# apache/incubator-predictionio

Hardware: NVIDIA H100
Metric: ALS iterations/sec (higher is better)
Workload: dtype f32

## Files before the change

### incubator-predictionio_b200/csrc/pio_als.cu

```cuda
#include "../../include/pio_als.h"

#include <cuda_runtime.h>
#include <dlfcn.h>
#include <math.h>
#include <nccl.h>
#include <stdarg.h>
#include <stdio.h>
#include <stdlib.h>
#include <string.h>

#include <chrono>
#include <algorithm>
#include <array>
#include <deque>
#include <exception>
#include <map>
#include <memory>
#include <mutex>
#include <string>
#include <type_traits>
#include <vector>

#include "als_kernels.cuh"
#include "als_mma_kernel.cuh"
#include "als_pair_kernel.cuh"
#define TC_NS tc
#define TC_NTEAM 2
#define TC_NCONV 5
#define TC_NGATHER 2
#define TC_NSTAGE 6
#define TC_NRAW 7
#include "als_tc_kernel.cuh"
#undef TC_NS
#undef TC_NTEAM
#undef TC_NCONV
#undef TC_NGATHER
#undef TC_NSTAGE
#undef TC_NRAW
#include "sort_scan.cuh"
#include "topk.cuh"
#include "score_plan.h"
#include "solve_plan.h"
#include "ids_encode.cuh"
#include "events_scan.cuh"
#include "events_fold.cuh"
#include "events_index.cuh"
#include "cooc.cuh"
#include "cooc_predict.cuh"
#include "popular.cuh"
#include "serve_merge.cuh"
#include "forest.cuh"
#include "eval_folds.cuh"
#include "cls_folds.cuh"

namespace pio {

static thread_local std::string g_create_error;

static int ceil_log2(uint64_t n) {
  int b = 0;
  while (b < 63 && (1ull << b) < n) ++b;
  return b < 1 ? 1 : b;
}
static int pad_rank(int k) { return k <= 16 ? 16 : k <= 32 ? 32 : k <= 64 ? 64 : 128; }

struct NcclApi {
  void* lib = nullptr;
  ncclResult_t (*GetUniqueId)(ncclUniqueId*) = nullptr;
  ncclResult_t (*CommInitRank)(ncclComm_t*, int, ncclUniqueId, int) = nullptr;
  ncclResult_t (*AllGather)(const void*, void*, size_t, ncclDataType_t, ncclComm_t, cudaStream_t) = nullptr;
  ncclResult_t (*AllReduce)(const void*, void*, size_t, ncclDataType_t, ncclRedOp_t, ncclComm_t, cudaStream_t) = nullptr;
  ncclResult_t (*Send)(const void*, size_t, ncclDataType_t, int, ncclComm_t, cudaStream_t) = nullptr;
  ncclResult_t (*Recv)(void*, size_t, ncclDataType_t, int, ncclComm_t, cudaStream_t) = nullptr;
  ncclResult_t (*GroupStart)() = nullptr;
  ncclResult_t (*GroupEnd)() = nullptr;
// ... 41 lines not shown
__global__ void head_flags_kernel(const uint64_t* keys, long long n, uint32_t* flag) {
  const long long e = (long long)blockIdx.x * blockDim.x + threadIdx.x;
  if (e < n) flag[e] = (e == 0 || keys[e] != keys[e - 1]) ? 1u : 0u;
}
__global__ void dedup_compact_kernel(const uint64_t* keys, const uint32_t* pay, const uint32_t* pos,
                                     long long n, int bits_i, const float* rating, const long long* ts,
                                     int mode, int* ou, int* oi, float* orr) {
  const long long e = (long long)blockIdx.x * blockDim.x + threadIdx.x;
  if (e >= n) return;
  const uint64_t key = keys[e];
  if (e > 0 && keys[e - 1] == key) return;
  float acc;
  if (mode == PIO_ALS_DEDUP_SUM) {
    acc = rating[pay[e]];
    for (long long t = e + 1; t < n && keys[t] == key; ++t) acc += rating[pay[t]];
  } else {
    long long best_t = ts ? ts[pay[e]] : 0;
    uint32_t best_p = pay[e];
    for (long long t = e + 1; t < n && keys[t] == key; ++t) {
      const uint32_t pp = pay[t];
      const long long tt = ts ? ts[pp] : 0;
      if (tt >= best_t) { best_t = tt; best_p = pp; }
    }
    acc = rating[best_p];
  }
  const uint32_t o = pos[e];
  ou[o] = (int)(key >> bits_i);
  oi[o] = (int)(key & ((1ull << bits_i) - 1ull));
  orr[o] = acc;
}
__global__ void degree_kernel(const int* u, const int* i, const float* r, long long n, uint32_t* du,
                              uint32_t* di, uint32_t* pu, uint32_t* pi) {
  const long long e = (long long)blockIdx.x * blockDim.x + threadIdx.x;
  if (e >= n) return;
  atomicAdd(&du[u[e]], 1u);
  atomicAdd(&di[i[e]], 1u);
  if (r[e] > 0.f) {
    atomicAdd(&pu[u[e]], 1u);
    atomicAdd(&pi[i[e]], 1u);
  }
}
__global__ void degree_keys_kernel(const uint32_t* deg, int n, uint64_t* keys, uint32_t* pay) {
  const int r = blockIdx.x * blockDim.x + threadIdx.x;
  if (r < n) {
    keys[r] = (uint64_t)(0xFFFFFFFFu - deg[r]);
    pay[r] = (uint32_t)r;
  }
}
__global__ void assign_internal_kernel(const uint32_t* order, int n, int W, int R, int* perm, int* inv, int* rpos,
                                       int* p2i) {
  const int p = blockIdx.x * blockDim.x + threadIdx.x;
  if (p >= n) return;
  const int row = (int)order[p];
  const int blk = p / W, pos = p % W;
  const int rk = (blk & 1) ? (W - 1 - pos) : pos;
  const int internal = rk * R + blk;
  perm[row] = internal;
  inv[internal] = row;
  rpos[row] = p;
  p2i[p] = internal;
}
__global__ void dest_mod_kernel(const int* u, long long n, int W, uint64_t* keys, uint32_t* pay) {
  const long long e = (long long)blockIdx.x * blockDim.x + threadIdx.x;
  if (e < n) {
    keys[e] = (uint64_t)((uint32_t)u[e] % (uint32_t)W);
    pay[e] = (uint32_t)e;
  }
}
__global__ void dest_owner_kernel(const int* rowext, long long n, const int* perm, int R, uint64_t* keys, uint32_t* pay) {
  const long long e = (long long)blockIdx.x * blockDim.x + threadIdx.x;
  if (e < n) {
    keys[e] = (uint64_t)(perm[rowext[e]] / R);
// ... 197 lines not shown
  cudaStream_t stream = nullptr;
  Side U, I;
  float* yty = nullptr;
  double* gram_partial = nullptr;
  double* gram_gsum = nullptr;
  const Side* gram_side = nullptr;
  cudaEvent_t ev_gram = nullptr;
  int gram_blocks = 0;
  int* d_fail = nullptr;
  int* d_counts = nullptr;
  unsigned* d_absmax = nullptr;
  long long* d_timing = nullptr;
  float* d_dbg = nullptr;
  size_t dbg_rows = 0;
  SolveSwitches sw;
  cudaStream_t aux = nullptr, comm_st = nullptr;
  cudaEvent_t ev_start = nullptr, ev_heavy = nullptr, ev_piece[8] = {}, ev_comm = nullptr;
  bool pieces_done = false;
  bool trace_on = false;
  std::chrono::steady_clock::time_point t_prev;
  unsigned char* srv_dev = nullptr;
  size_t srv_dev_cap = 0;
  unsigned char* srv_host = nullptr;
  unsigned char* srv_host_dev = nullptr;
  size_t srv_host_cap = 0;
  unsigned* srv_counter = nullptr;
  unsigned srv_seq = 0;
  bool serve_fused = true;
  bool score_blocked = true;
  bool serve_trace = false;
  float* tc_out = nullptr;
  size_t tc_out_rows = 0;
  bool have_ratings = false, have_init = false, trained = false;
  ncclComm_t comm = nullptr;
  std::string err;
  pio_als_stats st{};
  double phase_ms[8] = {0, 0, 0, 0, 0, 0, 0, 0};
  std::deque<EvPair> ev_pool;
  size_t ev_used = 0;
  std::mutex mu;
  int sm_count = 0;
};

namespace pio {

static int vfail(std::string& sink, int code, const char* fmt, va_list ap) {
  char buf[512];
  vsnprintf(buf, sizeof buf, fmt, ap);
  sink = buf;
  return code;
}
static int fail(pio_als_handle* h, int code, const char* fmt, ...) {
  va_list ap;
  va_start(ap, fmt);
  const int rc = vfail(h ? h->err : g_create_error, code, fmt, ap);
  va_end(ap);
  return rc;
}
static int fail_to(std::string* sink, int code, const char* fmt, ...) {
  va_list ap;
  va_start(ap, fmt);
  const int rc = vfail(*sink, code, fmt, ap);
  va_end(ap);
  return rc;
}
static void tmark(pio_als_handle* h, const char* what) {
// ... 250 lines not shown
  std::vector<unsigned char*> sendbufs(na, nullptr), recvbufs(na, nullptr);
  for (int a = 0; a < na; ++a) {
    if (!arrs[a].in) { *arrs[a].out = nullptr; continue; }
    CK(h, tmp.alloc(&sendbufs[a], (size_t)(n > 0 ? n : 1) * arrs[a].elem));
    CK(h, keep.alloc(&recvbufs[a], (size_t)(nrecv > 0 ? nrecv : 1) * arrs[a].elem));
    if (n > 0) {
      if (arrs[a].elem == 4)
        gather_by_index_kernel<uint32_t><<<nblk(n, 256), 256, 0, st>>>((const uint32_t*)arrs[a].in, vs, n, (uint32_t*)sendbufs[a]);
      else
        gather_by_index_kernel<uint64_t><<<nblk(n, 256), 256, 0, st>>>((const uint64_t*)arrs[a].in, vs, n, (uint64_t*)sendbufs[a]);
      LAUNCHED(h);
    }
    *arrs[a].out = recvbufs[a];
  }
  if (nc.GroupStart() != ncclSuccess) return fail(h, PIO_ALS_ERR_COMM, "ncclGroupStart failed");
  for (int a = 0; a < na; ++a) {
    if (!arrs[a].in) continue;
    for (int p = 0; p < W; ++p) {
      const long long sc = cnt[p], rc_ = all[(size_t)p * W + me];
      if (sc > 0 && nc.Send(sendbufs[a] + (size_t)off[p] * arrs[a].elem, (size_t)sc * arrs[a].elem, ncclInt8, p, h->comm, st) != ncclSuccess)
        return fail(h, PIO_ALS_ERR_COMM, "ncclSend failed");
      if (rc_ > 0 && nc.Recv(recvbufs[a] + (size_t)roff[p] * arrs[a].elem, (size_t)rc_ * arrs[a].elem, ncclInt8, p, h->comm, st) != ncclSuccess)
        return fail(h, PIO_ALS_ERR_COMM, "ncclRecv failed");
    }
  }
  if (nc.GroupEnd() != ncclSuccess) return fail(h, PIO_ALS_ERR_COMM, "ncclGroupEnd failed");
  CK(h, cudaStreamSynchronize(st));
  tmark(h, "  exchange: gather + send/recv");
  *n_out = nrecv;
  return PIO_ALS_OK;
}

static int ingest_device(pio_als_handle* h, const int* d_user, const int* d_item, const float* d_rating,
                         long long nnz, int dedup, const long long* d_ts, bool sharded) {
  cudaStream_t st = h->stream;
  const int W = h->cfg.world_size;
  sharded = sharded && W > 1;
  if (nnz <= 0 && !sharded)
    return fail(h, PIO_ALS_ERR_ARG, "ratings cannot be empty (the templates require(!ratings.take(1).isEmpty))");
  if (nnz < 0) return fail(h, PIO_ALS_ERR_ARG, "nnz < 0");
  if (nnz >= (1ll << 32)) return fail(h, PIO_ALS_ERR_ARG, "nnz must be < 2^32 per call");
  if (dedup < 0 || dedup > 2) return fail(h, PIO_ALS_ERR_ARG, "bad dedup_mode %d", dedup);
  free_side(h, h->U, true);
  free_side(h, h->I, true);
  h->have_ratings = false;
  Side& U = h->U;
  Side& I = h->I;
  U.n = h->cfg.n_users;
  I.n = h->cfg.n_items;
  U.R = (U.n + W - 1) / W;
  I.R = (I.n + W - 1) / W;
  U.n_internal = U.R * W;
  I.n_internal = I.R * W;
  U.bits = ceil_log2((uint64_t)U.n_internal);
  I.bits = ceil_log2((uint64_t)I.n_internal);

  h->trace_on = getenv("PIO_ALS_INGEST_TRACE") != nullptr;
  h->t_prev = std::chrono::steady_clock::now();
  auto mark = [&](const char* what) { tmark(h, what); };
  CK(h, cudaMemsetAsync(h->d_fail, 0, sizeof(int), st));
  if (nnz > 0) {
    validate_coo_kernel<<<nblk(nnz, 256), 256, 0, st>>>(d_user, d_item, nnz, U.n, I.n, h->d_fail);
    LAUNCHED(h);
  }
  int bad = 0;
  CK(h, cudaMemcpyAsync(&bad, h->d_fail, sizeof(int), cudaMemcpyDeviceToHost, st));
  CK(h, cudaStreamSynchronize(st));
  if (bad) return fail(h, PIO_ALS_ERR_ARG, "%d ratings have a user/item index out of range", bad);

  mark("validate");
  Scratch tmp(h->stream);
  const int* su = d_user;
  const int* si = d_item;
  const float* sr = d_rating;
  const long long* sts = d_ts;
  long long ns = nnz;
  if (sharded && dedup != PIO_ALS_DEDUP_NONE) {
    Scratch xs(h->stream);
    SortBufs sb;
    for (int i : {0, 1}) {
      CK(h, xs.alloc(&sb.k[i], (size_t)nnz));
      CK(h, xs.alloc(&sb.v[i], (size_t)nnz));
    }
    if (nnz > 0) {
      dest_mod_kernel<<<nblk(nnz, 256), 256, 0, st>>>(d_user, nnz, W, sb.keys(), sb.vals());
      LAUNCHED(h);
    }
    void *xu = nullptr, *xi = nullptr, *xr = nullptr, *xt = nullptr;
    XArr arrs[4] = {{d_user, &xu, 4}, {d_item, &xi, 4}, {d_rating, &xr, 4},
                    {dedup == PIO_ALS_DEDUP_KEEP_LAST ? (const void*)d_ts : nullptr, &xt, 8}};
    int rc = exchange_events(h, tmp, sb, nnz, arrs, 4, &ns);
    if (rc) return rc;
    su = (const int*)xu; si = (const int*)xi; sr = (const float*)xr; sts = (const long long*)xt;
  }

  mark("exchange by user residue");
  const int* cu = su;
  const int* ci = si;
  const float* cr = sr;
  long long n2 = ns;
  if (dedup != PIO_ALS_DEDUP_NONE && ns > 0) {
    Scratch ds(h->stream);
    SortBufs sb;
    for (int i : {0, 1}) {
      CK(h, ds.alloc(&sb.k[i], (size_t)ns));
      CK(h, ds.alloc(&sb.v[i], (size_t)ns));
    }
    const int bu = ceil_log2((uint64_t)U.n), bi = ceil_log2((uint64_t)I.n);
    make_keys_ext_kernel<<<nblk(ns, 256), 256, 0, st>>>(su, si, ns, bi, sb.keys(), sb.vals());
    LAUNCHED(h);
    CK(h, radix_sort_pairs(sb, (size_t)ns, bu + bi, st, &h->st.kernel_launches));
    const uint64_t* ks = sb.keys();
    const uint32_t* vs = sb.vals();
    uint32_t* flag = nullptr;
    CK(h, ds.alloc(&flag, (size_t)ns));
    head_flags_kernel<<<nblk(ns, 256), 256, 0, st>>>(ks, ns, flag);
    LAUNCHED(h);
    uint32_t last_flag = 0, last_pos = 0;
    CK(h, cudaMemcpyAsync(&last_flag, flag + ns - 1, sizeof(uint32_t), cudaMemcpyDeviceToHost, st));
    CK(h, scan_exclusive_u32(flag, flag, (size_t)ns, st, &h->st.kernel_launches));
    CK(h, cudaMemcpyAsync(&last_pos, flag + ns - 1, sizeof(uint32_t), cudaMemcpyDeviceToHost, st));
    CK(h, cudaStreamSynchronize(st));
    n2 = (long long)last_pos + last_flag;
    int *du_ = nullptr, *di_ = nullptr;
    float* dr_ = nullptr;
    CK(h, tmp.alloc(&du_, (size_t)n2));
    CK(h, tmp.alloc(&di_, (size_t)n2));
    CK(h, tmp.alloc(&dr_, (size_t)n2));
    dedup_compact_kernel<<<nblk(ns, 256), 256, 0, st>>>(ks, vs, flag, ns, bi, sr, sts, dedup, du_, di_, dr_);
    LAUNCHED(h);
    cu = du_;
    ci = di_;
    cr = dr_;
  }

  mark("dedup");
  for (Side* s : {&U, &I}) {
    CK(h, dalloc(h, &s->deg, (size_t)s->n));
    CK(h, dalloc(h, &s->npos, (size_t)s->n));
    CK(h, dalloc(h, &s->perm, (size_t)s->n));
    CK(h, dalloc(h, &s->inv, (size_t)s->n_internal));
    CK(h, dalloc(h, &s->rpos, (size_t)s->n));
    CK(h, dalloc(h, &s->p2i, (size_t)s->n));
    CK(h, cudaMemsetAsync(s->deg, 0, sizeof(uint32_t) * s->n, st));
    CK(h, cudaMemsetAsync(s->npos, 0, sizeof(uint32_t) * s->n, st));
  }
  if (n2 > 0) {
    degree_kernel<<<nblk(n2, 256), 256, 0, st>>>(cu, ci, cr, n2, U.deg, I.deg, U.npos, I.npos);
    LAUNCHED(h);
  }
  CK(h, cudaMemsetAsync(h->d_absmax + 1, 0, sizeof(unsigned), st));
  if (n2 > 0) {
    pr::abs_max_kernel<<<std::min(nblk(n2, 256), 4u * h->sm_count), 256, 0, st>>>(cr, n2, h->d_absmax + 1);
    LAUNCHED(h);
  }
  long long n2_global = n2;
  if (sharded) {
    NcclApi& nc = nccl_api();
    long long* d_n = nullptr;
    CK(h, tmp.alloc(&d_n, 1));
    CK(h, cudaMemcpyAsync(d_n, &n2, sizeof(long long), cudaMemcpyHostToDevice, st));
    if (nc.GroupStart() != ncclSuccess) return fail(h, PIO_ALS_ERR_COMM, "ncclGroupStart failed");
    for (Side* s : {&U, &I}) {
      if (nc.AllReduce(s->deg, s->deg, (size_t)s->n, ncclUint32, ncclSum, h->comm, st) != ncclSuccess ||
          nc.AllReduce(s->npos, s->npos, (size_t)s->n, ncclUint32, ncclSum, h->comm, st) != ncclSuccess)
        return fail(h, PIO_ALS_ERR_COMM, "ncclAllReduce (degrees) failed");
    }
    if (nc.AllReduce(d_n, d_n, 1, ncclInt64, ncclSum, h->comm, st) != ncclSuccess ||
        nc.AllReduce(h->d_absmax + 1, h->d_absmax + 1, 1, ncclUint32, ncclMax, h->comm, st) != ncclSuccess)
// ... 37 lines not shown
      XArr arrs[3] = {{j.rowext, &xrow, 4}, {j.colext, &xcol, 4}, {cr, &xr, 4}};
      long long ne = 0;
      rc = exchange_events(h, recv, sb, n2, arrs, 3, &ne);
      if (rc) return rc;
      mark("exchange by row owner");
      rc = build_side(h, *j.row, *j.col, (const int*)xrow, (const int*)xcol, (const float*)xr, ne, n2_global);
      if (rc) return rc;
      mark("build side");
    }
  }

  for (Side* s : {&U, &I}) {
    if (!s->F) {
      CK(h, dalloc(h, &s->F, (size_t)s->n_internal * h->KP));
      h->have_init = false;
    }
    CK(h, dalloc(h, &s->cand_ext, (size_t)s->n_internal));
    cand_ext_kernel<<<nblk(s->n_internal, 256), 256, 0, st>>>(s->inv, s->deg, s->n_internal, s->cand_ext);
    LAUNCHED(h);
  }
  h->have_init = false;
  CK(h, cudaStreamSynchronize(st));
  mark("factor buffers");
  h->st.n_users_active = U.n_active;
  h->st.n_items_active = I.n_active;
  if (W > 1) {
    h->st.n_users_active = -1;
    h->st.n_items_active = -1;
  }
  h->have_ratings = true;
  h->trained = false;
  return PIO_ALS_OK;
}

static int init_hash(pio_als_handle* h) {
  cudaStream_t st = h->stream;
  CK(h, cudaMemsetAsync(h->U.F, 0, sizeof(float) * (size_t)h->U.n_internal * h->KP, st));
  CK(h, cudaMemsetAsync(h->I.F, 0, sizeof(float) * (size_t)h->I.n_internal * h->KP, st));
  hash_init_kernel<<<nblk(h->U.n, 128), 128, 0, st>>>(h->U.n, h->cfg.rank, h->KP, (uint64_t)h->cfg.seed, 0, h->U.perm,
                                                      h->U.deg, h->U.F);
  LAUNCHED(h);
  hash_init_kernel<<<nblk(h->I.n, 128), 128, 0, st>>>(h->I.n, h->cfg.rank, h->KP, (uint64_t)h->cfg.seed, 1, h->I.perm,
                                                      h->I.deg, h->I.F);
  LAUNCHED(h);
  h->have_init = true;
  return PIO_ALS_OK;
}

using Cfg16 = SolveCfg<16, 4, 25, 8>;
using Cfg32 = SolveCfg<32, 8, 25, 4>;
using Cfg64 = SolveCfg<64, 8, 7, 8>;
using Cfg128 = SolveCfg<128, 8, 2, 9>;

static_assert(fp32_rows_per_cta(16) == Cfg16::NG && fp32_rows_per_cta(32) == Cfg32::NG &&
              fp32_rows_per_cta(64) == Cfg64::NG && fp32_rows_per_cta(128) == Cfg128::NG, "SolveCfg::NG");
static_assert(Cfg16::WARP_CHOL && Cfg32::WARP_CHOL && Cfg64::WARP_CHOL && Cfg128::LS_PARTIAL,
              "als_finish_kernel runs one warp per row below KP 128, and KP 128 takes the LS128 route");
static_assert(MMA_ROWS_PER_CTA == mm::WARPS, "mm::WARPS");
static_assert(TC_ROWS_PER_CTA == tc::Api::kPerCta && TC_SOLVE_ROWS_PER_CTA == tc::Api::kSolveWarps, "tc::Api");
static_assert(LS128_FINISH_ROWS_PER_CTA == FIN128_WARPS, "FIN128_WARPS");
static_assert(PART % Cfg16::CH == 0 && PART % Cfg32::CH == 0 && PART % Cfg64::CH == 0 && PART % Cfg128::CH == 0 &&
              PART % mm::CH == 0 && PART % tc::STAGE_RATINGS == 0, "PART");
static_assert(PAIR_PART % pr::CH == 0 && pr::CH == 8, "PAIR_PART and PIO_ALS_PART round to multiples of pr::CH");

static int ensure_dyn_smem(pio_als_handle* h, const void* kernel, size_t bytes, bool carveout = false) {
  struct Rec {
// ... 381 lines not shown
static int create_common(pio_als_handle* h) {
  int ndev = 0;
  cudaError_t ce = cudaGetDeviceCount(&ndev);
  if (ce != cudaSuccess || ndev == 0)
    return fail(nullptr, PIO_ALS_ERR_CUDA, "no CUDA device available (%s); this library has no CPU fallback",
                cudaGetErrorString(ce));
  if (h->cfg.device < 0 || h->cfg.device >= ndev) return fail(nullptr, PIO_ALS_ERR_ARG, "bad device %d", h->cfg.device);
  cudaDeviceProp pr;
  if (cudaGetDeviceProperties(&pr, h->cfg.device) != cudaSuccess) return fail(nullptr, PIO_ALS_ERR_CUDA, "cudaGetDeviceProperties");
  if (pr.major != 9 || pr.minor != 0)
    return fail(nullptr, PIO_ALS_ERR_CUDA, "device %d is sm_%d%d; this library is built for sm_90a (H100) only",
                h->cfg.device, pr.major, pr.minor);
  h->sm_count = pr.multiProcessorCount;
  h->st.sm_count = pr.multiProcessorCount;
  if (cudaSetDevice(h->cfg.device) != cudaSuccess) return fail(nullptr, PIO_ALS_ERR_CUDA, "cudaSetDevice");
  if (cudaStreamCreateWithFlags(&h->stream, cudaStreamNonBlocking) != cudaSuccess)
    return fail(nullptr, PIO_ALS_ERR_CUDA, "cudaStreamCreate");
  cudaMemPool_t pool;
  if (cudaDeviceGetDefaultMemPool(&pool, h->cfg.device) == cudaSuccess) {
    uint64_t thr = UINT64_MAX;
    cudaMemPoolSetAttribute(pool, cudaMemPoolAttrReleaseThreshold, &thr);
  }
  h->KP = pad_rank(h->cfg.rank);
  int prio_lo = 0, prio_hi = 0;
  cudaDeviceGetStreamPriorityRange(&prio_lo, &prio_hi);
  if (cudaStreamCreateWithFlags(&h->aux, cudaStreamNonBlocking) != cudaSuccess ||
      cudaStreamCreateWithPriority(&h->comm_st, cudaStreamNonBlocking, prio_hi) != cudaSuccess)
    return fail(nullptr, PIO_ALS_ERR_CUDA, "cudaStreamCreate");
  {
    cudaEvent_t* evs[5] = {&h->ev_start, &h->ev_heavy, &h->ev_comm, &h->ev_gram, nullptr};
    for (int i = 0; evs[i]; ++i)
      if (cudaEventCreateWithFlags(evs[i], cudaEventDisableTiming) != cudaSuccess) return fail(nullptr, PIO_ALS_ERR_CUDA, "cudaEventCreate");
    for (int i = 0; i < 8; ++i)
      if (cudaEventCreateWithFlags(&h->ev_piece[i], cudaEventDisableTiming) != cudaSuccess) return fail(nullptr, PIO_ALS_ERR_CUDA, "cudaEventCreate");
    if (const char* v = getenv("PIO_ALS_SERVE_FUSED")) h->serve_fused = atoi(v) != 0;
    if (const char* v = getenv("PIO_ALS_SERVE_TRACE")) h->serve_trace = atoi(v) != 0;
    if (const char* v = getenv("PIO_ALS_SCORE_BLOCKED")) h->score_blocked = atoi(v) != 0;
  }
  h->sw = read_solve_switches(getenv, h->KP, h->cfg.world_size);
  h->gram_blocks = GRAM_GROUPS * h->sm_count;
  if (cudaMallocAsync((void**)&h->yty, sizeof(float) * h->KP * h->KP, h->stream) != cudaSuccess ||
      cudaMallocAsync((void**)&h->gram_partial, sizeof(double) * (size_t)h->gram_blocks * h->KP * h->KP, h->stream) != cudaSuccess ||
      cudaMallocAsync((void**)&h->gram_gsum, sizeof(double) * (size_t)GRAM_GROUPS * h->KP * h->KP, h->stream) != cudaSuccess ||
      cudaMallocAsync((void**)&h->d_fail, sizeof(int), h->stream) != cudaSuccess ||
      cudaMallocAsync((void**)&h->d_counts, 4 * sizeof(int), h->stream) != cudaSuccess ||
      cudaMallocAsync((void**)&h->d_absmax, 2 * sizeof(unsigned), h->stream) != cudaSuccess)
    return fail(nullptr, PIO_ALS_ERR_CUDA, "device allocation failed");
  cudaMemsetAsync(h->yty, 0, sizeof(float) * h->KP * h->KP, h->stream);
  cudaMemsetAsync(h->d_fail, 0, sizeof(int), h->stream);
  return PIO_ALS_OK;
}

int pio_als_create(const pio_als_config* cfg, pio_als_handle** out) {
  if (!cfg || !out) return fail(nullptr, PIO_ALS_ERR_ARG, "null argument");
  *out = nullptr;
  if (cfg->abi_version != PIO_ALS_ABI_VERSION) return fail(nullptr, PIO_ALS_ERR_ARG, "abi_version mismatch");
  if (cfg->rank < 1 || cfg->rank > 128) return fail(nullptr, PIO_ALS_ERR_ARG, "rank must be in 1..128 (got %d)", cfg->rank);
  if (cfg->n_users < 1 || cfg->n_items < 1) return fail(nullptr, PIO_ALS_ERR_ARG, "n_users and n_items must be >= 1");
  if (cfg->world_size < 1 || cfg->world_rank < 0 || cfg->world_rank >= cfg->world_size)
    return fail(nullptr, PIO_ALS_ERR_ARG, "bad world_size/world_rank");
  if (!(cfg->lambda >= 0.0)) return fail(nullptr, PIO_ALS_ERR_ARG, "lambda must be >= 0");
  pio_als_handle* h = new pio_als_handle();
  h->cfg = *cfg;
  int rc = create_common(h);
  if (rc == PIO_ALS_OK && cfg->world_size > 1) {
    NcclApi& a = nccl_api();
    if (!a.ok) rc = fail(nullptr, PIO_ALS_ERR_COMM, "libnccl.so.2 not loadable");
    else {
      ncclUniqueId id;
      memcpy(&id, cfg->nccl_id, 128);
      ncclResult_t r = a.CommInitRank(&h->comm, cfg->world_size, id, cfg->world_rank);
      if (r != ncclSuccess) rc = fail(nullptr, PIO_ALS_ERR_COMM, "ncclCommInitRank failed: %s", a.GetErrorString ? a.GetErrorString(r) : "?");
    }
  }
  if (rc != PIO_ALS_OK) {
    pio_als_destroy(h);
    return rc;
  }
  *out = h;
  return PIO_ALS_OK;
}

void pio_als_destroy(pio_als_handle* h) {
  if (!h) return;
  if (h->stream) {
    cudaSetDevice(h->cfg.device);
    free_side(h, h->U, false);
    free_side(h, h->I, false);
    dfree(h, h->yty);
    dfree(h, h->gram_partial);
    dfree(h, h->gram_gsum);
    dfree(h, h->d_fail);
    dfree(h, h->d_counts);
    dfree(h, h->d_absmax);
    cudaStreamSynchronize(h->stream);
    if (h->tc_out) cudaFree(h->tc_out);
    if (h->d_dbg) cudaFree(h->d_dbg);
    if (h->d_timing) cudaFree(h->d_timing);
    for (auto& e : h->ev_pool) {
      cudaEventDestroy(e.a);
      cudaEventDestroy(e.b);
    }
    if (h->comm) nccl_api().CommDestroy(h->comm);
    if (h->ev_start) cudaEventDestroy(h->ev_start);
    if (h->ev_heavy) cudaEventDestroy(h->ev_heavy);
    if (h->ev_comm) cudaEventDestroy(h->ev_comm);
    if (h->ev_gram) cudaEventDestroy(h->ev_gram);
    for (int i = 0; i < 8; ++i)
      if (h->ev_piece[i]) cudaEventDestroy(h->ev_piece[i]);
    if (h->srv_dev) cudaFree(h->srv_dev);
    if (h->srv_host) cudaFreeHost(h->srv_host);
    if (h->srv_counter) cudaFree(h->srv_counter);
    if (h->aux) cudaStreamDestroy(h->aux);
    if (h->comm_st) cudaStreamDestroy(h->comm_st);
    cudaStreamDestroy(h->stream);
  }
  delete h;
}

static int set_ratings_impl(pio_als_handle* h, const int32_t* user, const int32_t* item, const float* rating, int64_t nnz,
                            int dedup_mode, const int64_t* ts, bool on_device, bool sharded) {
  if (!h) return PIO_ALS_ERR_ARG;
  const bool may_be_empty = sharded && h->cfg.world_size > 1;
  if (nnz < 0 || (nnz == 0 && !may_be_empty))
    return fail(h, PIO_ALS_ERR_ARG, "ratings cannot be empty (the templates require(!ratings.take(1).isEmpty))");
  if (nnz > 0 && (!user || !item || !rating)) return fail(h, PIO_ALS_ERR_ARG, "null rating arrays");
  if (nnz >= (1ll << 32)) return fail(h, PIO_ALS_ERR_ARG, "nnz must be < 2^32 per call");
  if (dedup_mode < 0 || dedup_mode > 2) return fail(h, PIO_ALS_ERR_ARG, "bad dedup_mode %d", dedup_mode);
  std::lock_guard<std::mutex> lk(h->mu);
  CK(h, cudaSetDevice(h->cfg.device));
  cudaStream_t st = h->stream;
  cudaEvent_t a, b;
  cudaEventCreate(&a);
  cudaEventCreate(&b);
  cudaEventRecord(a, st);
  int rc;
  {
    Scratch tmp(h->stream);
    const int *du = user, *di = item;
    const float* dr = rating;
    const long long* dts = (const long long*)ts;
    auto stage = [&]() -> int {
      if (on_device || nnz == 0) return PIO_ALS_OK;
      int *tu = nullptr, *ti = nullptr;
      float* tr = nullptr;
      long long* tt = nullptr;
      CK(h, tmp.alloc(&tu, (size_t)nnz));
      CK(h, tmp.alloc(&ti, (size_t)nnz));
      CK(h, tmp.alloc(&tr, (size_t)nnz));
      CK(h, cudaMemcpyAsync(tu, user, sizeof(int) * nnz, cudaMemcpyHostToDevice, st));
      CK(h, cudaMemcpyAsync(ti, item, sizeof(int) * nnz, cudaMemcpyHostToDevice, st));
      CK(h, cudaMemcpyAsync(tr, rating, sizeof(float) * nnz, cudaMemcpyHostToDevice, st));
      if (ts && dedup_mode == PIO_ALS_DEDUP_KEEP_LAST) {
        CK(h, tmp.alloc(&tt, (size_t)nnz));
        CK(h, cudaMemcpyAsync(tt, ts, sizeof(long long) * nnz, cudaMemcpyHostToDevice, st));
      }
      du = tu; di = ti; dr = tr; dts = tt;
      return PIO_ALS_OK;
    };
    rc = stage();
    if (rc == PIO_ALS_OK) rc = ingest_device(h, du, di, dr, nnz, dedup_mode, dts, sharded);
  }
  cudaEventRecord(b, st);
  cudaEventSynchronize(b);
  float ms = 0;
  cudaEventElapsedTime(&ms, a, b);
  h->st.last_ingest_ms = ms;
  cudaEventDestroy(a);
  cudaEventDestroy(b);
  return rc;
}

int pio_als_set_ratings_coo_device(pio_als_handle* h, const int32_t* d_user, const int32_t* d_item,
                                   const float* d_rating, int64_t nnz, int dedup_mode, const int64_t* d_ts) {
  return set_ratings_impl(h, d_user, d_item, d_rating, nnz, dedup_mode, d_ts, true, false);
}

int pio_als_set_ratings_coo(pio_als_handle* h, const int32_t* user, const int32_t* item, const float* rating,
                            int64_t nnz, int dedup_mode, const int64_t* ts) {
  return set_ratings_impl(h, user, item, rating, nnz, dedup_mode, ts, false, false);
}

int pio_als_set_ratings_coo_sharded(pio_als_handle* h, const int32_t* user, const int32_t* item, const float* rating,
                                    int64_t nnz_local, int dedup_mode, const int64_t* ts) {
  return set_ratings_impl(h, user, item, rating, nnz_local, dedup_mode, ts, false, true);
}

int pio_als_set_ratings_coo_sharded_device(pio_als_handle* h, const int32_t* d_user, const int32_t* d_item,
                                           const float* d_rating, int64_t nnz_local, int dedup_mode, const int64_t* d_ts) {
  return set_ratings_impl(h, d_user, d_item, d_rating, nnz_local, dedup_mode, d_ts, true, true);
}

__attribute__((visibility("default"))) int pio_als_debug_side(pio_als_handle* h, int side, int64_t scalars[11],
                                                              uint32_t* deg, uint32_t* npos, int32_t* perm, int32_t* inv,
// ... 17 lines not shown
      {nreg, s.nreg, sizeof(float) * (size_t)s.R},           {part_beg, s.part_beg, sizeof(int64_t) * (size_t)s.n_parts},
      {part_end, s.part_end, sizeof(int64_t) * (size_t)s.n_parts}};
  for (const auto& j : jobs)
    if (j.to && j.bytes) CK(h, cudaMemcpyAsync(j.to, j.from, j.bytes, cudaMemcpyDeviceToHost, st));
  if (row_part_ptr && s.n_heavy > 0) std::copy(s.h_row_part_ptr.begin(), s.h_row_part_ptr.end(), row_part_ptr);
  CK(h, cudaStreamSynchronize(st));
  return PIO_ALS_OK;
}

int pio_als_set_init(pio_als_handle* h, const float* user_factors, const float* item_factors) {
  if (!h) return PIO_ALS_ERR_ARG;
  std::lock_guard<std::mutex> lk(h->mu);
  if (!h->have_ratings) return fail(h, PIO_ALS_ERR_STATE, "set_init before set_ratings");
  if (!user_factors) return fail(h, PIO_ALS_ERR_ARG, "user_factors is null");
  CK(h, cudaSetDevice(h->cfg.device));
  cudaStream_t st = h->stream;
  const int k = h->cfg.rank;
  struct { Side* s; const float* f; } jobs[2] = {{&h->U, user_factors}, {&h->I, item_factors}};
  for (auto& j : jobs) {
    CK(h, cudaMemsetAsync(j.s->F, 0, sizeof(float) * (size_t)j.s->n_internal * h->KP, st));
    if (!j.f) continue;
    float* tmp = nullptr;
    CK(h, dalloc(h, &tmp, (size_t)j.s->n * k));
    CK(h, cudaMemcpyAsync(tmp, j.f, sizeof(float) * (size_t)j.s->n * k, cudaMemcpyHostToDevice, st));
    scatter_init_kernel<<<nblk((long long)j.s->n * h->KP, 256), 256, 0, st>>>(tmp, j.s->n, k, h->KP, j.s->perm, j.s->deg, j.s->F);
    LAUNCHED(h);
    dfree(h, tmp);
  }
  CK(h, cudaStreamSynchronize(st));
  h->have_init = true;
  return PIO_ALS_OK;
}

int pio_als_run(pio_als_handle* h, int n_iters) {
  if (!h) return PIO_ALS_ERR_ARG;
  std::lock_guard<std::mutex> lk(h->mu);
  if (!h->have_ratings) return fail(h, PIO_ALS_ERR_STATE, "run before set_ratings");
  if (n_iters < 0) return fail(h, PIO_ALS_ERR_ARG, "n_iters < 0");
  CK(h, cudaSetDevice(h->cfg.device));
  if (!h->have_init) {
    if (h->cfg.init_mode == PIO_ALS_INIT_HASH) {
      int rc = init_hash(h);
      if (rc) return rc;
    } else {
      return fail(h, PIO_ALS_ERR_STATE, "no initial factors: call pio_als_set_init or use PIO_ALS_INIT_HASH");
    }
  }
  cudaStream_t st = h->stream;
  h->ev_used = 0;
  CK(h, cudaMemsetAsync(h->d_fail, 0, sizeof(int), st));
  EvPair& tot = next_ev(h, -1);
  cudaEventRecord(tot.a, st);
  h->gram_side = nullptr;
  for (int it = 0; it < n_iters; ++it) {
    int rc = half_step(h, h->I, h->U, true);
    if (rc) return rc;
    rc = half_step(h, h->U, h->I, it + 1 < n_iters);
    if (rc) return rc;
  }
  cudaEventRecord(tot.b, st);
  int nfail = 0;
  CK(h, cudaMemcpyAsync(&nfail, h->d_fail, sizeof(int), cudaMemcpyDeviceToHost, st));
  CK(h, cudaStreamSynchronize(st));
  double ms[EV_NKIND] = {0, 0, 0, 0};
  float t = 0;
  for (size_t i = 0; i < h->ev_used; ++i) {
    EvPair& e = h->ev_pool[i];
    cudaEventElapsedTime(&t, e.a, e.b);
    if (e.kind >= 0) ms[e.kind] += t;
    else h->st.last_run_ms = t;
  }
  h->st.last_solve_ms = ms[EV_SOLVE] + ms[EV_SOLVE_USER];
  h->phase_ms[0] = ms[EV_SOLVE];
  h->phase_ms[1] = ms[EV_SOLVE_USER];
  h->phase_ms[2] = ms[EV_GRAM];
  h->phase_ms[3] = ms[EV_COMM];
  h->phase_ms[6] = (double)n_iters;
  h->st.last_gram_ms = ms[EV_GRAM];
  h->st.last_comm_ms = ms[EV_COMM];
  h->trained = true;
  if (nfail)
    return fail(h, PIO_ALS_ERR_NUMERIC, "%d normal equations were not positive definite (MLlib: dppsv info != 0)", nfail);
  return PIO_ALS_OK;
}

int pio_als_get_phase_ms(pio_als_handle* h, double out[8]) {
  if (!h || !out) return PIO_ALS_ERR_ARG;
  std::lock_guard<std::mutex> lk(h->mu);
  for (int i = 0; i < 8; ++i) out[i] = h->phase_ms[i];
  out[4] = phase_code(h->I.plan.kernel);
  out[5] = phase_code(h->U.plan.kernel);
  return PIO_ALS_OK;
}

int pio_als_get_factors(pio_als_handle* h, float* user_out, float* item_out, uint8_t* user_has, uint8_t* item_has) {
  if (!h) return PIO_ALS_ERR_ARG;
  std::lock_guard<std::mutex> lk(h->mu);
  if (!h->have_ratings && !h->trained) return fail(h, PIO_ALS_ERR_STATE, "no model");
  CK(h, cudaSetDevice(h->cfg.device));
  cudaStream_t st = h->stream;
  const int k = h->cfg.rank;
  struct { Side* s; float* f; uint8_t* has; } jobs[2] = {{&h->U, user_out, user_has}, {&h->I, item_out, item_has}};
  for (auto& j : jobs) {
    if (j.f) {
      float* tmp = nullptr;
      CK(h, dalloc(h, &tmp, (size_t)j.s->n * k));
      gather_factors_kernel<<<nblk((long long)j.s->n * k, 256), 256, 0, st>>>(j.s->F, j.s->n, k, h->KP, j.s->perm, tmp);
      LAUNCHED(h);
      CK(h, cudaMemcpyAsync(j.f, tmp, sizeof(float) * (size_t)j.s->n * k, cudaMemcpyDeviceToHost, st));
      dfree(h, tmp);
    }
    if (j.has) {
      uint8_t* tmp = nullptr;
      CK(h, dalloc(h, &tmp, (size_t)j.s->n));
      has_kernel<<<nblk(j.s->n, 256), 256, 0, st>>>(j.s->deg, j.s->n, tmp);
      LAUNCHED(h);
      CK(h, cudaMemcpyAsync(j.has, tmp, (size_t)j.s->n, cudaMemcpyDeviceToHost, st));
      dfree(h, tmp);
    }
  }
  CK(h, cudaStreamSynchronize(st));
  return PIO_ALS_OK;
}

int pio_als_train(pio_als_handle* h, const int32_t* user, const int32_t* item, const float* rating, int64_t nnz,
                  int dedup_mode, const int64_t* ts, const float* user_init, const float* item_init, int n_iters,
                  float* user_out, float* item_out, uint8_t* user_has, uint8_t* item_has) {
  int rc = pio_als_set_ratings_coo(h, user, item, rating, nnz, dedup_mode, ts);
  if (rc) return rc;
  if (user_init) {
    rc = pio_als_set_init(h, user_init, item_init);
    if (rc) return rc;
  }
  rc = pio_als_run(h, n_iters);
  if (rc) return rc;
  return pio_als_get_factors(h, user_out, item_out, user_has, item_has);
}

}

namespace pio {
static int serve_reserve(pio_als_handle* h, size_t dev_bytes, size_t host_bytes) {
  if (h->srv_dev_cap < dev_bytes) {
    CK(h, cudaStreamSynchronize(h->stream));
    if (h->srv_dev) cudaFree(h->srv_dev);
    h->srv_dev = nullptr;
    h->srv_dev_cap = 0;
    CK(h, cudaMalloc((void**)&h->srv_dev, dev_bytes));
    h->srv_dev_cap = dev_bytes;
  }
  if (h->srv_host_cap < host_bytes) {
    CK(h, cudaStreamSynchronize(h->stream));
    if (h->srv_host) cudaFreeHost(h->srv_host);
    h->srv_host = nullptr;
    h->srv_host_cap = 0;
    CK(h, cudaHostAlloc((void**)&h->srv_host, host_bytes, cudaHostAllocMapped));
    CK(h, cudaHostGetDevicePointer((void**)&h->srv_host_dev, h->srv_host, 0));
    h->srv_host_cap = host_bytes;
  }
  return PIO_ALS_OK;
}
static inline size_t al256(size_t x) { return (x + 255) & ~(size_t)255; }

struct ArenaLayout {
  size_t bytes = 0;
  size_t take(size_t n) {
    const size_t at = bytes;
    bytes = al256(bytes + n);
    return at;
// ... 4548 lines not shown
```

Before: 35.58.

## Pipeline host-device staging of ratings and factors through pinned ring buffers

Replaces the monolithic pageable H2D copies of the COO ratings with chunked copies through a pinned ring buffer on a separate copy stream, filled by a multithreaded memcpy team, so validation overlaps with transfer. Factor output copies also go through the ring, and in train the item factors are copied out on the copy stream while the final user half-step runs. The degree kernel aggregates warp-level duplicate indices with match_any before issuing atomics. This adds threads, pinned memory and extra events in exchange for overlapping transfer with compute; the ALS iteration loop itself is unchanged.

```diff
diff --git a/incubator-predictionio_b200/csrc/host_stage.h b/incubator-predictionio_b200/csrc/host_stage.h
--- /dev/null
+++ b/incubator-predictionio_b200/csrc/host_stage.h
@@ -0,0 +1,98 @@
+#pragma once
+
+#include <stdint.h>
+#include <stdlib.h>
+#include <string.h>
+
+#include <condition_variable>
+#include <mutex>
+#include <thread>
+#include <vector>
+
+namespace pio {
+
+struct StageSwitches {
+  long long chunk = 1ll << 20;
+  int depth = 2;
+  int threads = 4;
+};
+
+template <class Env>
+inline StageSwitches read_stage_switches(Env env) {
+  StageSwitches s;
+  const char* v;
+  if ((v = env("PIO_ALS_STAGE_CHUNK")) && atoll(v) >= 1) s.chunk = atoll(v) < (1ll << 26) ? atoll(v) : (1ll << 26);
+  if ((v = env("PIO_ALS_STAGE_DEPTH")) && atoi(v) >= 2 && atoi(v) <= 8) s.depth = atoi(v);
+  if ((v = env("PIO_ALS_STAGE_THREADS")) && atoi(v) >= 1 && atoi(v) <= 32) s.threads = atoi(v);
+  return s;
+}
+
+struct CopyPiece {
+  void* dst;
+  const void* src;
+  size_t bytes;
+};
+
+class CopyTeam {
+ public:
+  explicit CopyTeam(int n) : n_(n < 1 ? 1 : n) {
+    for (int t = 1; t < n_; ++t) th_.emplace_back([this, t] { worker(t); });
+  }
+  CopyTeam(const CopyTeam&) = delete;
+  CopyTeam& operator=(const CopyTeam&) = delete;
+  ~CopyTeam() {
+    {
+      std::lock_guard<std::mutex> lk(m_);
+      quit_ = true;
+    }
+    go_.notify_all();
+    for (std::thread& t : th_) t.join();
+  }
+  void run(const CopyPiece* p, int np) {
+    {
+      std::lock_guard<std::mutex> lk(m_);
+      p_ = p;
+      np_ = np;
+      left_ = n_ - 1;
+      ++gen_;
+    }
+    go_.notify_all();
+    part(0);
+    std::unique_lock<std::mutex> lk(m_);
+    done_.wait(lk, [&] { return left_ == 0; });
+  }
+
+ private:
+  void part(int t) const {
+    for (int k = 0; k < np_; ++k) {
+      const size_t b = p_[k].bytes;
+      const size_t lo = (b * t / n_) & ~(size_t)63;
+      const size_t hi = t + 1 == n_ ? b : (b * (t + 1) / n_) & ~(size_t)63;
+      if (hi > lo) memcpy((char*)p_[k].dst + lo, (const char*)p_[k].src + lo, hi - lo);
+    }
+  }
+  void worker(int t) {
+    uint64_t seen = 0;
+    for (;;) {
+      {
+        std::unique_lock<std::mutex> lk(m_);
+        go_.wait(lk, [&] { return quit_ || gen_ != seen; });
+        if (quit_) return;
+        seen = gen_;
+      }
+      part(t);
+      std::lock_guard<std::mutex> lk(m_);
+      if (--left_ == 0) done_.notify_one();
+    }
+  }
+  const int n_;
+  std::vector<std::thread> th_;
+  std::mutex m_;
+  std::condition_variable go_, done_;
+  const CopyPiece* p_ = nullptr;
+  int np_ = 0, left_ = 0;
+  uint64_t gen_ = 0;
+  bool quit_ = false;
+};
+
+}
diff --git a/incubator-predictionio_b200/csrc/pio_als.cu b/incubator-predictionio_b200/csrc/pio_als.cu
--- a/incubator-predictionio_b200/csrc/pio_als.cu
+++ b/incubator-predictionio_b200/csrc/pio_als.cu
@@ -41,6 +41,7 @@
 #include "topk.cuh"
 #include "score_plan.h"
 #include "solve_plan.h"
+#include "host_stage.h"
 #include "ids_encode.cuh"
 #include "events_scan.cuh"
 #include "events_fold.cuh"
@@ -148,12 +149,20 @@
 __global__ void degree_kernel(const int* u, const int* i, const float* r, long long n, uint32_t* du,
                               uint32_t* di, uint32_t* pu, uint32_t* pi) {
   const long long e = (long long)blockIdx.x * blockDim.x + threadIdx.x;
+  const unsigned act = __ballot_sync(0xffffffffu, e < n);
   if (e >= n) return;
-  atomicAdd(&du[u[e]], 1u);
-  atomicAdd(&di[i[e]], 1u);
-  if (r[e] > 0.f) {
-    atomicAdd(&pu[u[e]], 1u);
-    atomicAdd(&pi[i[e]], 1u);
+  const int lane = threadIdx.x & 31;
+  const int uu = u[e], ii = i[e];
+  const unsigned pos = __ballot_sync(act, r[e] > 0.f);
+  const unsigned mu = __match_any_sync(act, uu);
+  if (lane == __ffs(mu) - 1) {
+    atomicAdd(&du[uu], (unsigned)__popc(mu));
+    if (pos & mu) atomicAdd(&pu[uu], (unsigned)__popc(pos & mu));
+  }
+  const unsigned mi = __match_any_sync(act, ii);
+  if (lane == __ffs(mi) - 1) {
+    atomicAdd(&di[ii], (unsigned)__popc(mi));
+    if (pos & mi) atomicAdd(&pi[ii], (unsigned)__popc(pos & mi));
   }
 }
 __global__ void degree_keys_kernel(const uint32_t* deg, int n, uint64_t* keys, uint32_t* pay) {
@@ -417,6 +426,13 @@
   float* tc_out = nullptr;
   size_t tc_out_rows = 0;
   bool have_ratings = false, have_init = false, trained = false;
+  StageSwitches stage;
+  cudaStream_t cp_st = nullptr;
+  cudaEvent_t ring_ev[8] = {}, ev_cp = nullptr, ev_items_final = nullptr;
+  unsigned char* ring = nullptr;
+  size_t ring_slot = 0;
+  float* d_out = nullptr;
+  uint8_t* d_out_has = nullptr;
   ncclComm_t comm = nullptr;
   std::string err;
   pio_als_stats st{};
@@ -733,7 +749,8 @@
 }
 
 static int ingest_device(pio_als_handle* h, const int* d_user, const int* d_item, const float* d_rating,
-                         long long nnz, int dedup, const long long* d_ts, bool sharded) {
+                         long long nnz, int dedup, const long long* d_ts, bool sharded, bool validated,
+                         cudaEvent_t ratings_ready) {
   cudaStream_t st = h->stream;
   const int W = h->cfg.world_size;
   sharded = sharded && W > 1;
@@ -759,8 +776,13 @@
   h->trace_on = getenv("PIO_ALS_INGEST_TRACE") != nullptr;
   h->t_prev = std::chrono::steady_clock::now();
   auto mark = [&](const char* what) { tmark(h, what); };
-  CK(h, cudaMemsetAsync(h->d_fail, 0, sizeof(int), st));
-  if (nnz > 0) {
+  auto ratings = [&]() -> int {
+    if (ratings_ready) CK(h, cudaStreamWaitEvent(st, ratings_ready, 0));
+    ratings_ready = nullptr;
+    return PIO_ALS_OK;
+  };
+  if (!validated) CK(h, cudaMemsetAsync(h->d_fail, 0, sizeof(int), st));
+  if (nnz > 0 && !validated) {
     validate_coo_kernel<<<nblk(nnz, 256), 256, 0, st>>>(d_user, d_item, nnz, U.n, I.n, h->d_fail);
     LAUNCHED(h);
   }
@@ -788,6 +810,7 @@
       LAUNCHED(h);
     }
     void *xu = nullptr, *xi = nullptr, *xr = nullptr, *xt = nullptr;
+    if (int rc = ratings()) return rc;
     XArr arrs[4] = {{d_user, &xu, 4}, {d_item, &xi, 4}, {d_rating, &xr, 4},
                     {dedup == PIO_ALS_DEDUP_KEEP_LAST ? (const void*)d_ts : nullptr, &xt, 8}};
     int rc = exchange_events(h, tmp, sb, nnz, arrs, 4, &ns);
@@ -828,6 +851,7 @@
     CK(h, tmp.alloc(&du_, (size_t)n2));
     CK(h, tmp.alloc(&di_, (size_t)n2));
     CK(h, tmp.alloc(&dr_, (size_t)n2));
+    if (int rc = ratings()) return rc;
     dedup_compact_kernel<<<nblk(ns, 256), 256, 0, st>>>(ks, vs, flag, ns, bi, sr, sts, dedup, du_, di_, dr_);
     LAUNCHED(h);
     cu = du_;
@@ -836,6 +860,7 @@
   }
 
   mark("dedup");
+  if (int rc = ratings()) return rc;
   for (Side* s : {&U, &I}) {
     CK(h, dalloc(h, &s->deg, (size_t)s->n));
     CK(h, dalloc(h, &s->npos, (size_t)s->n));
@@ -939,6 +964,152 @@
   h->trained = false;
   return PIO_ALS_OK;
 }
+
+static bool host_pinned(const void* p) {
+  cudaPointerAttributes a;
+  if (cudaPointerGetAttributes(&a, p) != cudaSuccess) {
+    cudaGetLastError();
+    return false;
+  }
+  return a.type == cudaMemoryTypeHost;
+}
+
+static int ring_reserve(pio_als_handle* h) {
+  if (h->ring) return PIO_ALS_OK;
+  const size_t slot = (size_t)h->stage.chunk * (2 * sizeof(int) + sizeof(float) + sizeof(long long));
+  CK(h, cudaHostAlloc((void**)&h->ring, slot * h->stage.depth, cudaHostAllocDefault));
+  h->ring_slot = slot;
+  return PIO_ALS_OK;
+}
+
+struct CopyMark {
+  pio_als_handle* h;
+  ~CopyMark() { cudaEventRecord(h->ev_cp, h->cp_st); }
+};
+
+static int stage_h2d(pio_als_handle* h, Scratch& tmp, const void* const* src, const size_t* elem, int na, long long nnz,
+                     void** dst) {
+  cudaStream_t st = h->stream, cp = h->cp_st;
+  bool pinned[4], any_pageable = false;
+  for (int a = 0; a < na; ++a) {
+    CK(h, tmp.alloc((unsigned char**)&dst[a], (size_t)nnz * elem[a]));
+    pinned[a] = host_pinned(src[a]);
+    any_pageable |= !pinned[a];
+  }
+  std::unique_ptr<CopyTeam> team;
+  if (any_pageable) {
+    const int rc = ring_reserve(h);
+    if (rc) return rc;
+    team.reset(new CopyTeam(h->stage.threads));
+  }
+  CK(h, cudaMemsetAsync(h->d_fail, 0, sizeof(int), st));
+  CK(h, cudaEventRecord(h->ev_cp, st));
+  CK(h, cudaStreamWaitEvent(cp, h->ev_cp, 0));
+  CopyMark mark{h};
+  const long long C = h->stage.chunk;
+  const int D = h->stage.depth;
+  const int* du = (const int*)dst[0];
+  const int* di = (const int*)dst[1];
+  long long k = 0;
+  for (int a0 : {0, 2}) {
+    const int a1 = a0 == 0 ? 2 : na;
+    for (long long off = 0; off < nnz; off += C, ++k) {
+      const long long len = std::min(C, nnz - off);
+      const int slot = (int)(k % D);
+      unsigned char* ring = any_pageable ? h->ring + slot * h->ring_slot : nullptr;
+      const void* from[4];
+      CopyPiece pc[4];
+      int np = 0;
+      if (any_pageable) CK(h, cudaEventSynchronize(h->ring_ev[slot]));
+      for (int a = a0; a < a1; ++a) {
+        const unsigned char* s = (const unsigned char*)src[a] + off * elem[a];
+        if (pinned[a]) {
+          from[a] = s;
+          continue;
+        }
+        pc[np++] = {ring, s, len * elem[a]};
+        from[a] = ring;
+        ring += C * elem[a];
+      }
+      if (np) team->run(pc, np);
+      for (int a = a0; a < a1; ++a)
+        CK(h, cudaMemcpyAsync((unsigned char*)dst[a] + off * elem[a], from[a], len * elem[a], cudaMemcpyHostToDevice, cp));
+      CK(h, cudaEventRecord(h->ring_ev[slot], cp));
+      if (a0 == 0) {
+        CK(h, cudaStreamWaitEvent(st, h->ring_ev[slot], 0));
+        validate_coo_kernel<<<nblk(len, 256), 256, 0, st>>>(du + off, di + off, len, h->cfg.n_users, h->cfg.n_items,
+                                                            h->d_fail);
+        LAUNCHED(h);
+      }
+    }
+  }
+  return PIO_ALS_OK;
+}
+
+static int copy_to_host(pio_als_handle* h, void* dst, const void* src, size_t bytes, cudaStream_t cs,
+                        std::unique_ptr<CopyTeam>& team) {
+  if (bytes == 0) return PIO_ALS_OK;
+  if (host_pinned(dst)) {
+    CK(h, cudaMemcpyAsync(dst, src, bytes, cudaMemcpyDeviceToHost, cs));
+    return PIO_ALS_OK;
+  }
+  int rc = ring_reserve(h);
+  if (rc) return rc;
+  if (!team) team.reset(new CopyTeam(h->stage.threads));
+  const size_t S = h->ring_slot;
+  const long long D = h->stage.depth, n = (long long)((bytes + S - 1) / S);
+  auto issue = [&](long long c) -> int {
+    const int slot = (int)(c % D);
+    CK(h, cudaEventSynchronize(h->ring_ev[slot]));
+    CK(h, cudaMemcpyAsync(h->ring + slot * S, (const char*)src + c * S, std::min(S, bytes - (size_t)c * S),
+                          cudaMemcpyDeviceToHost, cs));
+    CK(h, cudaEventRecord(h->ring_ev[slot], cs));
+    return PIO_ALS_OK;
+  };
+  for (long long c = 0; c < n && c < D; ++c)
+    if ((rc = issue(c))) return rc;
+  for (long long c = 0; c < n; ++c) {
+    const int slot = (int)(c % D);
+    CK(h, cudaEventSynchronize(h->ring_ev[slot]));
+    const CopyPiece pc{(char*)dst + c * S, h->ring + slot * S, std::min(S, bytes - (size_t)c * S)};
+    team->run(&pc, 1);
+    if (c + D < n && (rc = issue(c + D))) return rc;
+  }
+  return PIO_ALS_OK;
+}
+
+static int out_reserve(pio_als_handle* h) {
+  const size_t rows = (size_t)h->cfg.n_users + h->cfg.n_items;
+  if (!h->d_out_has) CK(h, cudaMalloc((void**)&h->d_out_has, rows));
+  if (!h->d_out) CK(h, cudaMalloc((void**)&h->d_out, sizeof(float) * rows * h->cfg.rank));
+  return PIO_ALS_OK;
+}
+
+static int side_out(pio_als_handle* h, const Side& s, float* f, uint8_t* has, cudaStream_t cs,
+                    std::unique_ptr<CopyTeam>& team) {
+  const int k = h->cfg.rank;
+  const size_t row0 = &s == &h->U ? 0 : (size_t)h->cfg.n_users;
+  if (f) {
+    float* d = h->d_out + row0 * k;
+    gather_factors_kernel<<<nblk((long long)s.n * k, 256), 256, 0, cs>>>(s.F, s.n, k, h->KP, s.perm, d);
+    LAUNCHED(h);
+    const int rc = copy_to_host(h, f, d, sizeof(float) * (size_t)s.n * k, cs, team);
+    if (rc) return rc;
+  }
+  if (has) {
+    uint8_t* d = h->d_out_has + row0;
+    has_kernel<<<nblk(s.n, 256), 256, 0, cs>>>(s.deg, s.n, d);
+    LAUNCHED(h);
+    return copy_to_host(h, has, d, (size_t)s.n, cs, team);
+  }
+  return PIO_ALS_OK;
+}
+
+struct ItemsOut {
+  float* f;
+  uint8_t* has;
+  std::unique_ptr<CopyTeam>* team;
+};
 
 static int init_hash(pio_als_handle* h) {
   cudaStream_t st = h->stream;
@@ -1386,12 +1557,20 @@
     for (int i = 0; evs[i]; ++i)
       if (cudaEventCreateWithFlags(evs[i], cudaEventDisableTiming) != cudaSuccess) return fail(nullptr, PIO_ALS_ERR_CUDA, "cudaEventCreate");
     for (int i = 0; i < 8; ++i)
-      if (cudaEventCreateWithFlags(&h->ev_piece[i], cudaEventDisableTiming) != cudaSuccess) return fail(nullptr, PIO_ALS_ERR_CUDA, "cudaEventCreate");
+      if (cudaEventCreateWithFlags(&h->ev_piece[i], cudaEventDisableTiming) != cudaSuccess ||
+          cudaEventCreateWithFlags(&h->ring_ev[i], cudaEventDisableTiming) != cudaSuccess)
+        return fail(nullptr, PIO_ALS_ERR_CUDA, "cudaEventCreate");
+    if (cudaEventCreateWithFlags(&h->ev_cp, cudaEventDisableTiming) != cudaSuccess ||
+        cudaEventCreateWithFlags(&h->ev_items_final, cudaEventDisableTiming) != cudaSuccess)
+      return fail(nullptr, PIO_ALS_ERR_CUDA, "cudaEventCreate");
+    if (cudaStreamCreateWithFlags(&h->cp_st, cudaStreamNonBlocking) != cudaSuccess)
+      return fail(nullptr, PIO_ALS_ERR_CUDA, "cudaStreamCreate");
     if (const char* v = getenv("PIO_ALS_SERVE_FUSED")) h->serve_fused = atoi(v) != 0;
     if (const char* v = getenv("PIO_ALS_SERVE_TRACE")) h->serve_trace = atoi(v) != 0;
     if (const char* v = getenv("PIO_ALS_SCORE_BLOCKED")) h->score_blocked = atoi(v) != 0;
   }
   h->sw = read_solve_switches(getenv, h->KP, h->cfg.world_size);
+  h->stage = read_stage_switches(getenv);
   h->gram_blocks = GRAM_GROUPS * h->sm_count;
   if (cudaMallocAsync((void**)&h->yty, sizeof(float) * h->KP * h->KP, h->stream) != cudaSuccess ||
       cudaMallocAsync((void**)&h->gram_partial, sizeof(double) * (size_t)h->gram_blocks * h->KP * h->KP, h->stream) != cudaSuccess ||
@@ -1448,6 +1627,15 @@
     dfree(h, h->d_counts);
     dfree(h, h->d_absmax);
     cudaStreamSynchronize(h->stream);
+    if (h->cp_st) cudaStreamSynchronize(h->cp_st);
+    if (h->ring) cudaFreeHost(h->ring);
+    if (h->d_out) cudaFree(h->d_out);
+    if (h->d_out_has) cudaFree(h->d_out_has);
+    for (int i = 0; i < 8; ++i)
+      if (h->ring_ev[i]) cudaEventDestroy(h->ring_ev[i]);
+    if (h->ev_cp) cudaEventDestroy(h->ev_cp);
+    if (h->ev_items_final) cudaEventDestroy(h->ev_items_final);
+    if (h->cp_st) cudaStreamDestroy(h->cp_st);
     if (h->tc_out) cudaFree(h->tc_out);
     if (h->d_dbg) cudaFree(h->d_dbg);
     if (h->d_timing) cudaFree(h->d_timing);
@@ -1494,26 +1682,22 @@
     const int *du = user, *di = item;
     const float* dr = rating;
     const long long* dts = (const long long*)ts;
-    auto stage = [&]() -> int {
-      if (on_device || nnz == 0) return PIO_ALS_OK;
-      int *tu = nullptr, *ti = nullptr;
-      float* tr = nullptr;
-      long long* tt = nullptr;
-      CK(h, tmp.alloc(&tu, (size_t)nnz));
-      CK(h, tmp.alloc(&ti, (size_t)nnz));
-      CK(h, tmp.alloc(&tr, (size_t)nnz));
-      CK(h, cudaMemcpyAsync(tu, user, sizeof(int) * nnz, cudaMemcpyHostToDevice, st));
-      CK(h, cudaMemcpyAsync(ti, item, sizeof(int) * nnz, cudaMemcpyHostToDevice, st));
-      CK(h, cudaMemcpyAsync(tr, rating, sizeof(float) * nnz, cudaMemcpyHostToDevice, st));
-      if (ts && dedup_mode == PIO_ALS_DEDUP_KEEP_LAST) {
-        CK(h, tmp.alloc(&tt, (size_t)nnz));
-        CK(h, cudaMemcpyAsync(tt, ts, sizeof(long long) * nnz, cudaMemcpyHostToDevice, st));
-      }
-      du = tu; di = ti; dr = tr; dts = tt;
-      return PIO_ALS_OK;
-    };
-    rc = stage();
-    if (rc == PIO_ALS_OK) rc = ingest_device(h, du, di, dr, nnz, dedup_mode, dts, sharded);
+    const bool staged = !on_device && nnz > 0;
+    rc = PIO_ALS_OK;
+    if (staged) {
+      const bool with_ts = ts && dedup_mode == PIO_ALS_DEDUP_KEEP_LAST;
+      const void* src[4] = {user, item, rating, ts};
+      const size_t elem[4] = {sizeof(int), sizeof(int), sizeof(float), sizeof(long long)};
+      void* dst[4] = {nullptr, nullptr, nullptr, nullptr};
+      rc = stage_h2d(h, tmp, src, elem, with_ts ? 4 : 3, nnz, dst);
+      du = (const int*)dst[0];
+      di = (const int*)dst[1];
+      dr = (const float*)dst[2];
+      dts = (const long long*)dst[3];
+    }
+    if (rc == PIO_ALS_OK)
+      rc = ingest_device(h, du, di, dr, nnz, dedup_mode, dts, sharded, staged, staged ? h->ev_cp : nullptr);
+    if (staged) cudaStreamWaitEvent(st, h->ev_cp, 0);
   }
   cudaEventRecord(b, st);
   cudaEventSynchronize(b);
@@ -1597,9 +1781,9 @@
   return PIO_ALS_OK;
 }
 
-int pio_als_run(pio_als_handle* h, int n_iters) {
-  if (!h) return PIO_ALS_ERR_ARG;
-  std::lock_guard<std::mutex> lk(h->mu);
+}
+
+static int run_iters(pio_als_handle* h, int n_iters, ItemsOut* items) {
   if (!h->have_ratings) return fail(h, PIO_ALS_ERR_STATE, "run before set_ratings");
   if (n_iters < 0) return fail(h, PIO_ALS_ERR_ARG, "n_iters < 0");
   CK(h, cudaSetDevice(h->cfg.device));
@@ -1620,10 +1804,16 @@
   for (int it = 0; it < n_iters; ++it) {
     int rc = half_step(h, h->I, h->U, true);
     if (rc) return rc;
+    if (items && it + 1 == n_iters) CK(h, cudaEventRecord(h->ev_items_final, st));
     rc = half_step(h, h->U, h->I, it + 1 < n_iters);
     if (rc) return rc;
   }
   cudaEventRecord(tot.b, st);
+  if (items && n_iters > 0) {
+    CK(h, cudaStreamWaitEvent(h->cp_st, h->ev_items_final, 0));
+    const int rc = side_out(h, h->I, items->f, items->has, h->cp_st, *items->team);
+    if (rc) return rc;
+  }
   int nfail = 0;
   CK(h, cudaMemcpyAsync(&nfail, h->d_fail, sizeof(int), cudaMemcpyDeviceToHost, st));
   CK(h, cudaStreamSynchronize(st));
@@ -1649,6 +1839,14 @@
   return PIO_ALS_OK;
 }
 
+extern "C" {
+
+int pio_als_run(pio_als_handle* h, int n_iters) {
+  if (!h) return PIO_ALS_ERR_ARG;
+  std::lock_guard<std::mutex> lk(h->mu);
+  return run_iters(h, n_iters, nullptr);
+}
+
 int pio_als_get_phase_ms(pio_als_handle* h, double out[8]) {
   if (!h || !out) return PIO_ALS_ERR_ARG;
   std::lock_guard<std::mutex> lk(h->mu);
@@ -1663,29 +1861,13 @@
   std::lock_guard<std::mutex> lk(h->mu);
   if (!h->have_ratings && !h->trained) return fail(h, PIO_ALS_ERR_STATE, "no model");
   CK(h, cudaSetDevice(h->cfg.device));
-  cudaStream_t st = h->stream;
-  const int k = h->cfg.rank;
-  struct { Side* s; float* f; uint8_t* has; } jobs[2] = {{&h->U, user_out, user_has}, {&h->I, item_out, item_has}};
-  for (auto& j : jobs) {
-    if (j.f) {
-      float* tmp = nullptr;
-      CK(h, dalloc(h, &tmp, (size_t)j.s->n * k));
-      gather_factors_kernel<<<nblk((long long)j.s->n * k, 256), 256, 0, st>>>(j.s->F, j.s->n, k, h->KP, j.s->perm, tmp);
-      LAUNCHED(h);
-      CK(h, cudaMemcpyAsync(j.f, tmp, sizeof(float) * (size_t)j.s->n * k, cudaMemcpyDeviceToHost, st));
-      dfree(h, tmp);
-    }
-    if (j.has) {
-      uint8_t* tmp = nullptr;
-      CK(h, dalloc(h, &tmp, (size_t)j.s->n));
-      has_kernel<<<nblk(j.s->n, 256), 256, 0, st>>>(j.s->deg, j.s->n, tmp);
-      LAUNCHED(h);
-      CK(h, cudaMemcpyAsync(j.has, tmp, (size_t)j.s->n, cudaMemcpyDeviceToHost, st));
-      dfree(h, tmp);
-    }
-  }
-  CK(h, cudaStreamSynchronize(st));
-  return PIO_ALS_OK;
+  int rc = out_reserve(h);
+  if (rc) return rc;
+  std::unique_ptr<CopyTeam> team;
+  rc = side_out(h, h->U, user_out, user_has, h->stream, team);
+  if (!rc) rc = side_out(h, h->I, item_out, item_has, h->stream, team);
+  CK(h, cudaStreamSynchronize(h->stream));
+  return rc;
 }
 
 int pio_als_train(pio_als_handle* h, const int32_t* user, const int32_t* item, const float* rating, int64_t nnz,
@@ -1697,9 +1879,19 @@
     rc = pio_als_set_init(h, user_init, item_init);
     if (rc) return rc;
   }
-  rc = pio_als_run(h, n_iters);
+  std::lock_guard<std::mutex> lk(h->mu);
+  CK(h, cudaSetDevice(h->cfg.device));
+  rc = out_reserve(h);
   if (rc) return rc;
-  return pio_als_get_factors(h, user_out, item_out, user_has, item_has);
+  std::unique_ptr<CopyTeam> team;
+  ItemsOut items{item_out, item_has, &team};
+  const bool early = n_iters > 0 && (item_out || item_has);
+  rc = run_iters(h, n_iters, early ? &items : nullptr);
+  if (!rc) rc = side_out(h, h->U, user_out, user_has, h->stream, team);
+  if (!rc && !early) rc = side_out(h, h->I, item_out, item_has, h->stream, team);
+  CK(h, cudaStreamSynchronize(h->stream));
+  CK(h, cudaStreamSynchronize(h->cp_st));
+  return rc;
 }
 
 }
```

New measurement: 35.53 (median of 6 runs). About the same (-0.1%).
